# genome/breakdancer

Hardware: AMD Instinct MI355X
Metric: read-pairs/s, records resident in HBM -> scored SV table (SURVEY 8d timing i); end to end from BAM: config.timings.bam_to_table (vs_baseline is taken there) (higher is better)
Workload: dtype int32

## Files before the change

breakdancer_amd/csrc/bdx_api.hip:

```cpp
#include <hip/hip_runtime.h>

#include <algorithm>
#include <atomic>
#include <functional>
#include <memory>
#include <chrono>
#include <cmath>
#include <cstdio>
#include <cstddef>
#include <cstring>
#include <string>
#include <thread>
#include <unordered_map>
#include <utility>
#include <vector>

#include "../../include/bdx.h"
#include "bdx_buf.h"
#include "bdx_dev.h"
#include "bdx_k3.h"
#include "bdx_shard.h"
#include "bdx_scan.h"
#include "bdx_walk.h"
#include "bdx_bam_dev.h"
// ... 15 lines not shown
    DevBuf b_groups;
    DevBuf b_r_rec, b_r_pk, b_out_deg, b_parts, b_rs, b_slot, b_members, b_own, b_lib_stage, b_cn_stage, b_t_lambda, b_t_k, b_ws6;
    DevBuf b_sv_src, b_dlists, b_ltail, b_ins, b_member_ids;
    DevBuf b_sv_out, b_lib_index_out, b_lib_pairs_out, b_cn_key_out, b_cn_value_out, b_ltail_out, b_sv_key;
    PinBuf h_regs, h_pk, h_groups, h_counts0, h_counts2, h_sv_out, h_lib_index, h_lib_pairs, h_cn_key, h_cn_value, h_ltail_dev;
};

constexpr int kNumStages = 12;
enum StageMs { kMsClassify, kMsCompact, kMsCut, kMsJoinAssemble, kMsGroupsWait, kMsHostWalk, kMsFinish, kMsRun, kMsTableWait, kMsMerge, kMsScores };
enum ReadyWord { kPass1Ready, kGroupsReady, kTableReady, kRegionsReady };
constexpr int kK1MaxGrid = 8192;
constexpr uint32_t kK1EventPeriod = 4;

}

struct bdx_ctx {
    int device = 0;
    Stream stream;
    Stream copy_stream;
    bdx_opts opts{};
    std::vector<bdx_lib> libs;
    int nlibs = 0, nbams = 0, ntids = 0, nkeys = 0, w0 = 0;
    std::string err;

    ReadsSoA d{};
    size_t n = 0, cap = 0;
    bool adopted = false;
    DevBuf b_tid, b_pos, b_mtid, b_mpos, b_isize, b_flag, b_qlen, b_mapq, b_lib, b_bam, b_key, b_check;
    bool groups_in_hbm = false;
    bool use_check = false;

    DevBuf b_libs, b_cls, b_tile_tot, b_tile_pre, b_tile_mono, b_blk_cnt, b_cnt, b_p1, b_fold, b_stash, b_chunk_tot, b_counts;
    DevBuf b_lib_mean, b_kdens;
    PinBuf h_p1, h_cnt, h_counts, h_terms;
    PinBuf h_hs_rec, h_hs_aux, h_hs_lists, h_printed;
    StageBufs sb;
    PinBuf h_flags;
    PinBuf h_count;
    uint32_t seq = 0;
    int dbg_no_stash = 0, dbg_max_chunks = 0, dbg_ins_plain = 0, dbg_gather_walk = 0, dbg_regions_copy = 0, dbg_asm_plain = 0, dbg_depth_plain = 0;
    uint32_t lb_seq = 0;
    float k1_ms_last = 0;
    bool k1_timed = false;
    bool stage_timing = false;
    bool poll = true;
    bool materialized = true;
    bool rows_packed = false;
    uint32_t n_sv_total = 0, n_groups_total = 0, n_terms_total = 0, n_cn_total = 0;
    Event ev_groups, ev_regions;
    int big_walk_mode = -1;
    int64_t last_big_groups = -1;
    FinalizeParams fp_deferred{};
    bool finalize2_deferred = false;
    bool bucketed_join = false;
    bool host_walk_only = false;
    K6Arrays k6{};
    const GroupRec* k6_in_groups = nullptr;
    const uint32_t* k6_in_goff = nullptr;
    bool force_direct_join = false;
    uint32_t k6_cap = 0;
    const RegionRec* k6_r_rec = nullptr;
    const uint32_t* k6_r_pk = nullptr;
    uint8_t* k6_taint = nullptr;
    bool table_in_hbm = false;

    bool ran = false;
    Pass1 p1{};
    StageCounts counts{};
    std::vector<uint32_t> cnt;
    std::vector<uint32_t> cnt_local;
    uint32_t g_covered = 0;
    int32_t g_window = 0;
    uint32_t ntiles = 0, tstride = 0;
    Compact cp{};
    K3Arrays k3{};
    K4Arrays k4{};
    std::vector<double> log_tail;
    bool collect_support = false;
    std::vector<uint32_t> ov_cnt;
    uint32_t ov_covered = 0;
    bool replayed = false;
    bool use_stash = false;
    std::atomic<int> sizing{0};
    std::string sizing_err;
    std::vector<uint32_t> sup_off;
    std::vector<uint64_t> sup_idx;
    std::vector<uint8_t> sup_flag;
    std::vector<float> seqcov, lib_density, key_density;
    std::vector<HostRegion> regions;
    std::vector<uint32_t> r_pk;
    const HostRegion* reg = nullptr;
    size_t nreg = 0;
    const uint32_t* rpk = nullptr;
    std::vector<GroupPart> parts;
    WalkResult walk;
    std::unique_ptr<WalkScratch, void (*)(WalkScratch*)> walk_scratch{nullptr, walk_scratch_free};
    uint32_t n_printed = 0;
    uint32_t n_sv_host = 0;
    int speculate = 2;
    int spec_test = 0;
    uint32_t last_na = 0;
    size_t last_n = 0;
    uint32_t count_chunks = 0;
    uint32_t na_alloc = 0;
    bool region_of_fused = false;
    uint32_t join_table_clean = 0;
// ... 510 lines not shown
    }
    launch_kd_apply(p, flag, mask, s);
    HIPCHK(c, hipGetLastError());
    if (h.nwork) {
        HIPCHK(c, hipMemcpyAsync(&h, p.cnt, sizeof(h), hipMemcpyDeviceToHost, s));
        HIPCHK(c, hipStreamSynchronize(s));
        if (h.nlist != h.nwork) return fail(c, BDX_EINTERNAL, "duplicate marking: the work list does not hold the candidates that were counted");
        k.release_long();
    }
    *marked += h.marked; *groups += h.groups;
    return BDX_OK;
}

int mark_duplicates(bdx_ctx* c) {
    if (c->dup_done) return BDX_OK;
    c->dup_marked = 0; c->dup_groups = 0;
    hipStream_t s = c->stream;
    if (c->adopted && (const void*)c->d.flag != c->b_flag.p) {
        HIPCHK(c, c->b_flag.ensure(c->n * 2));
        HIPCHK(c, hipMemcpyAsync(c->b_flag.p, c->d.flag, c->n * 2, hipMemcpyDeviceToDevice, s));
        c->d.flag = c->b_flag.as<uint16_t>();
    }
    KdParams p{};
    p.tid = c->d.tid; p.pos = c->d.pos; p.mtid = c->d.mtid; p.mpos = c->d.mpos; p.flag = c->d.flag;
    p.lib = c->nlibs > 1 ? c->d.lib : nullptr;
    p.key = c->d.key; p.n = c->n;
    size_t ns = 0;
    BDX_TRY(upload_key_segs(c, &ns));
    if (ns) {
        p.nseg = (int)ns;
        p.seg_begin = c->b_seg.as<uint64_t>();
        p.seg_ptr = (const uint64_t* const*)(c->b_seg.as<uint64_t>() + ns + 1);
    }
    BDX_TRY(kd_run(c, p, c->kd, (uint16_t*)c->d.flag, nullptr, s, &c->dup_marked, &c->dup_groups));
    c->dup_done = true;
    return BDX_OK;
}

int pass1_prepare(bdx_ctx* c, uint32_t tiles_cap) {
    HIPCHK(c, hipSetDevice(c->device));
    hipStream_t s = c->stream;
    const int nlibs = c->nlibs, nbams = c->nbams, nkeys = c->nkeys;
    const int ncols = 2 + nkeys, ncnt = nlibs * kNumFlags + nlibs + nbams;
    const uint32_t tstride = (uint32_t)round_up(std::max<uint32_t>(tiles_cap, 16), 16);
    c->tstride = tstride;
    c->k1_cap_tiles = tiles_cap;
    c->k1_done = 0;
    HIPCHK(c, c->b_cls.ensure(std::max<size_t>((size_t)tiles_cap * kTile, 16)));
    c->use_stash = !c->dbg_no_stash && nkeys <= kStashKeys;
    if (c->use_stash) HIPCHK(c, c->b_stash.ensure(std::max<size_t>((size_t)tiles_cap * kStashCap * sizeof(StashRec), 64)));
    HIPCHK(c, c->b_tile_tot.ensure((size_t)ncols * tstride * 4));
    HIPCHK(c, c->b_tile_pre.ensure((size_t)ncols * tstride * 4));
    HIPCHK(c, c->b_tile_mono.ensure((size_t)nbams * tstride * sizeof(MonoRec)));
    HIPCHK(c, c->b_blk_cnt.ensure((size_t)kCntCopies * ncnt * 4));
    HIPCHK(c, c->b_cnt.ensure((size_t)ncnt * 4));
    HIPCHK(c, c->b_p1.ensure(sizeof(Pass1)));
    HIPCHK(c, c->h_p1.ensure(sizeof(Pass1)));
    HIPCHK(c, c->h_cnt.ensure((size_t)ncnt * 4));
    HIPCHK(c, c->h_counts.ensure(sizeof(StageCounts)));
    HIPCHK(c, c->b_counts.ensure(sizeof(StageCounts)));
    HIPCHK(c, c->h_count.ensure((size_t)kMaxChunks * 8));
    const size_t w_tot = (size_t)ncols * tstride, w_mono = (size_t)nbams * tstride * sizeof(MonoRec) / 4;
    if (w_tot > 0xFFFFFFFFull || w_mono > 0xFFFFFFFFull) {
        HIPCHK(c, hipMemsetAsync(c->b_tile_tot.p, 0, w_tot * 4, s));
        HIPCHK(c, hipMemsetAsync(c->b_tile_mono.p, 0xFF, w_mono * 4, s));
    }
    InitList il{};
    int k = 0;
    auto add = [&](void* p, size_t words, uint32_t value) { il.ptr[k] = (uint32_t*)p; il.words[k] = (uint32_t)words; il.value[k] = value; ++k; };
    if (w_tot <= 0xFFFFFFFFull && w_mono <= 0xFFFFFFFFull) { add(c->b_tile_tot.p, w_tot, 0u); add(c->b_tile_mono.p, w_mono, 0xFFFFFFFFu); }
    add(c->b_blk_cnt.p, (size_t)kCntCopies * ncnt, 0u);
    add(c->b_p1.p, sizeof(Pass1) / 4, 0u);
    add(c->b_counts.p, sizeof(StageCounts) / 4, 0u);
    il.n = k;
    launch_init(il, s);
    return BDX_OK;
}

int pass1_classify(bdx_ctx* c, uint32_t upto, bool timed) {
    hipStream_t s = c->stream;
    if (upto <= c->k1_done) return BDX_OK;
    K1Params k1{};
    k1.r = c->d; k1.n = c->n; k1.ntiles = upto; k1.tstride = c->tstride; k1.tile0 = c->k1_done;
    k1.nlibs = c->nlibs; k1.nbams = c->nbams; k1.nkeys = c->nkeys;
    k1.max_sd = c->opts.max_sd; k1.opt_t = c->opts.transchr_rearrange; k1.opt_l = c->opts.illumina_long_insert;
    k1.libs = c->b_libs.as<DevLib>(); k1.cls = c->b_cls.as<uint8_t>(); k1.tile_tot = c->b_tile_tot.as<uint32_t>();
    k1.tile_mono = c->b_tile_mono.as<MonoRec>();
    k1.blk_cnt = c->b_blk_cnt.as<uint32_t>();
    k1.stash = c->use_stash ? c->b_stash.as<StashRec>() : nullptr;
    const uint32_t span = upto - c->k1_done;
    const int grid1 = (int)std::min<uint32_t>((span + kWaves - 1) / kWaves, (uint32_t)kK1MaxGrid);
    launch_k1(k1, grid1, k1_lds_bytes(c->nlibs, c->nbams, c->nkeys), s, timed ? c->ev[0] : nullptr, timed ? c->ev[1] : nullptr);
    c->k1_done = upto;
    return BDX_OK;
}

struct Pass1Launch {
    uint32_t na_cap = 0;
    bool defer_second = false;
    bool post_count = false;
};
int pass1_finalize(bdx_ctx* c, const Pass1Launch& opt) {
    const int nlibs = c->nlibs, nbams = c->nbams, nkeys = c->nkeys;
    const int ncols = 2 + nkeys, ncnt = nlibs * kNumFlags + nlibs + nbams;
    const uint32_t ntiles = c->ntiles;
    FinalizeParams fp{};
    fp.ntiles = ntiles; fp.tstride = c->tstride; fp.nblk = 0;
    fp.nfold = std::max<uint32_t>(1, std::min<uint32_t>(64, (ntiles + 1023) / 1024));
    HIPCHK(c, c->b_fold.ensure((size_t)nbams * fp.nfold * sizeof(MonoRec)));
    fp.fold_part = c->b_fold.as<MonoRec>();
    fp.nlibs = nlibs; fp.nbams = nbams; fp.nkeys = nkeys; fp.ncols = ncols; fp.ncnt = ncnt; fp.w0 = c->w0;
    fp.tile_tot = c->b_tile_tot.as<uint32_t>(); fp.tile_pre = c->b_tile_pre.as<uint32_t>(); fp.tile_mono = c->b_tile_mono.as<MonoRec>();
    {
        const uint32_t nsuper = (ntiles + kK2TilesPerWave - 1) / kK2TilesPerWave;
        const uint32_t round = 4096;
        const uint32_t rounds = std::max<uint32_t>(1, (nsuper + round - 1) / round);
        const uint32_t max_chunks = c->dbg_max_chunks > 0 ? (uint32_t)std::min(c->dbg_max_chunks, (int)kMaxChunks) : (uint32_t)kMaxChunks;
        fp.chunk_super = round * ((rounds + max_chunks - 1) / max_chunks);
        fp.nchunk = std::max<uint32_t>(1, (nsuper + fp.chunk_super - 1) / fp.chunk_super);
        HIPCHK(c, c->b_chunk_tot.ensure((size_t)ncols * kMaxChunks * 8));
        fp.chunk_tot = c->b_chunk_tot.as<uint32_t>();
        fp.chunk_base = fp.chunk_tot + (size_t)ncols * kMaxChunks;
    }
    fp.blk_cnt = c->b_blk_cnt.as<uint32_t>(); fp.cnt = c->b_cnt.as<uint32_t>(); fp.p1 = c->b_p1.as<Pass1>();
    HIPCHK(c, c->b_kdens.ensure(64 * 4));
    fp.libs = c->b_libs.as<DevLib>(); fp.cn_lib = c->opts.cn_lib; fp.key_density = c->b_kdens.as<float>();
    fp.cnt_host = c->h_cnt.as<uint32_t>(); fp.p1_host = c->h_p1.as<Pass1>();
    memset(c->h_p1.p, 0, sizeof(Pass1));
    HIPCHK(c, c->h_flags.ensure(64));
    ++c->seq;
    fp.flag_host = c->h_flags.as<uint32_t>(); fp.flag_value = c->seq;
    fp.na_cap = opt.na_cap;
    fp.count_host = opt.post_count && c->poll ? c->h_count.as<uint64_t>() : nullptr; fp.count_stamp = c->seq;
    c->count_chunks = fp.count_host ? fp.nchunk : 0;
    c->fp_deferred = fp;
    c->finalize2_deferred = opt.defer_second;
    launch_finalize(fp, c->stream, !opt.defer_second);
    return BDX_OK;
}

int do_pass1(bdx_ctx* c, const Pass1Launch& opt) {
    HIPCHK(c, hipSetDevice(c->device));
    hipStream_t s = c->stream;
    if (c->n >= ((size_t)1 << 32)) return fail(c, BDX_ELIMIT, "more than 2^32 - 1 reads in one context (read indices and the prefix counters are 32-bit)");
    const uint32_t ntiles = (uint32_t)((c->n + kTile - 1) / kTile);
    c->ntiles = ntiles;
    c->ran = false; c->replayed = false;
    c->cls_n = (size_t)-1;
    c->na_alloc = 0;
    c->regions.clear(); c->r_pk.clear(); c->parts.clear();
    c->reg = nullptr; c->nreg = 0; c->rpk = nullptr;
    c->walk.clear();
    if (!c->walk_scratch) c->walk_scratch.reset(walk_scratch_new());
    c->n_printed = 0;
    memset(&c->counts, 0, sizeof(c->counts));
    for (float& m : c->stage_ms) m = 0;

    if (c->copy_pending) {
        HIPCHK(c, hipStreamWaitEvent(s, c->ev_copy, 0));
        c->copy_pending = false;
    }
    if (!(c->k1_live && c->k1_cap_tiles >= ntiles)) {
        BDX_TRY(pass1_prepare(c, ntiles));
    }
    c->k1_live = false;
    if (c->mark_dup && c->k1_done == 0) {
        BDX_TRY(mark_duplicates(c));
    }
    const bool time_k1 = (c->stage_timing || c->seq % kK1EventPeriod == 0) && c->k1_done == 0 && ntiles > 0;
    BDX_TRY(pass1_classify(c, ntiles, time_k1));
    BDX_TRY(pass1_finalize(c, opt));
    c->k1_timed = time_k1;
    return BDX_OK;
}

int wait_pass1(bdx_ctx* c) {
    const int ncnt = c->nlibs * kNumFlags + c->nlibs + c->nbams;
    BDX_TRY(await_ready(c, kPass1Ready, nullptr, "the pass-1 record did not arrive: its kernel was not launched", true));
    c->p1 = *c->h_p1.as<Pass1>();
    c->cnt_local.assign(c->h_cnt.as<uint32_t>(), c->h_cnt.as<uint32_t>() + ncnt);
    if (c->k1_timed) {
        float ms = 0;
        if (hipEventElapsedTime(&ms, c->ev[0], c->ev[1]) == hipSuccess) c->k1_ms_last = ms;
    }
    c->stage_ms[kMsClassify] = c->k1_ms_last;
    if (c->p1.n_anom > kMaxAnomalous) return fail(c, BDX_ELIMIT, "more than 2^31 anomalous reads in one context");
    if (!c->na_alloc && c->p1.n_anom) c->na_alloc = (uint32_t)std::min<uint64_t>(with_headroom(c->p1.n_anom), kMaxAnomalous);
    c->cls_n = c->n;
    return BDX_OK;
}

int32_t window_from(const bdx_ctx* c, const uint32_t* cnt, uint32_t covered) {
    int W = c->w0;
    for (int i = 0; i < c->nlibs; ++i) {
        const int nd = (int)(cnt[i * kNumFlags + F_LARGE] + cnt[i * kNumFlags + F_SMALL]);
        const int tmp = nd > 0 ? (int)((float)covered / (float)nd) : 50;
        W = std::min(W, tmp);
    }
    return W;
}

int set_pass1(bdx_ctx* c, const uint32_t* cnt, uint32_t covered, int32_t window, bool upload) {
    const int nlibs = c->nlibs, nkeys = c->nkeys;
    const int ncnt = nlibs * kNumFlags + nlibs + c->nbams;
    c->cnt.assign(cnt, cnt + ncnt);
    c->g_covered = covered;
    c->g_window = window;
    const uint32_t* lib_cnt = c->cnt.data() + nlibs * kNumFlags;
    const uint32_t* bam_cnt = lib_cnt + nlibs;
    c->seqcov.assign(nlibs, 0.f);
    c->lib_density.assign(nlibs, 0.f);
    c->key_density.assign(nkeys, 0.000001f);
    for (int i = 0; i < nlibs; ++i) {
        float covg = 0;
        if (lib_cnt[i] != 0 && covered != 0) covg = float(lib_cnt[i]) * c->libs[i].readlens / covered;
        c->seqcov[i] = covg;
        float dens = 0.000001f;
        if (c->opts.cn_lib) {
            if (lib_cnt[i] != 0) dens = float(lib_cnt[i]) / covered;
        } else {
            dens = float(bam_cnt[c->libs[i].bam_index]) / covered;
        }
        c->lib_density[i] = dens;
        c->key_density[c->opts.cn_lib ? i : c->libs[i].bam_index] = dens;
    }
    struct { uint32_t covered; int32_t window; } hdr{covered, window};
    static_assert(offsetof(Pass1, covered_ref_len) == 0 && offsetof(Pass1, window) == 4, "Pass1 header layout");
    if (upload) {
        HIPCHK(c, hipMemcpyAsync(c->b_p1.p, &hdr, sizeof(hdr), hipMemcpyHostToDevice, c->stream));
        HIPCHK(c, hipStreamSynchronize(c->stream));
    }
// ... 93 lines not shown
    SZCHK(b.b_cn_stage.ensure(cap * (size_t)d.nkeys * sizeof(CnStage) + 16));
    SZCHK(b.b_t_lambda.ensure((size_t)k.term * 8)); SZCHK(b.b_t_k.ensure((size_t)k.term * 4));
    if (d.table_in_hbm) {
        SZCHK(b.b_sv_out.ensure((size_t)k.sv * sizeof(SvOut))); SZCHK(b.b_sv_key.ensure((size_t)k.sv * 8));
        SZCHK(b.b_lib_index_out.ensure((size_t)k.term * 4)); SZCHK(b.b_lib_pairs_out.ensure((size_t)k.term * 4));
        SZCHK(b.b_cn_key_out.ensure((size_t)k.cn * 4 + 16)); SZCHK(b.b_cn_value_out.ensure((size_t)k.cn * 4 + 16));
        SZCHK(b.b_ltail_out.ensure((size_t)k.term * 8));
    } else {
        SZCHK(b.h_sv_out.ensure((size_t)k.sv * sizeof(SvOut)));
        SZCHK(b.h_lib_index.ensure((size_t)k.term * 4)); SZCHK(b.h_lib_pairs.ensure((size_t)k.term * 4));
        SZCHK(b.h_cn_key.ensure((size_t)k.cn * 4 + 16)); SZCHK(b.h_cn_value.ensure((size_t)k.cn * 4 + 16));
        SZCHK(b.h_ltail_dev.ensure((size_t)k.term * 8));
    }
    SZCHK(b.h_counts2.ensure(sizeof(StageCounts)));
    SZCHK(b.b_sv_src.ensure((size_t)k.sv * 16)); SZCHK(b.b_ltail.ensure((size_t)k.term * 8));
    SZCHK(b.b_dlists.ensure((size_t)k.term * 4 + (size_t)k.cn * 8 + 64));
    SZCHK(b.b_ins.ensure(k.p2 * 12 + (size_t)k.sv * 8 + ((size_t)k.sv + 1) * 16 + k.nsort * 12 + k.nsort * 4 * kK6RankSlices + 64));
    SZCHK(size_zero_once(b.b_ws6, 4 * (scan_grid((uint32_t)cap, 1) + 1) * 8, s));
    return BDX_OK;
}

int do_compact(bdx_ctx* c) {
    HIPCHK(c, hipSetDevice(c->device));
    hipStream_t s = c->stream;
    const int nkeys = c->nkeys;
    const uint32_t na = c->na_alloc;
    if (c->stage_timing) HIPCHK(c, hipEventRecord(c->ev[2], s));
    Compact& cp = c->cp;
    cp = Compact{};
    c->k3 = K3Arrays{};
    if (na) {
        const StageDims dm = stage_dims(c, na);
        BDX_TRY(size_compact(c->sb, dm, &c->err));
        const StageBufs& b = c->sb;
        cp.tid = b.b_c_tid.as<int32_t>(); cp.pos = b.b_c_pos.as<int32_t>(); cp.isize = b.b_c_isize.as<int32_t>();
        cp.meta = b.b_c_meta.as<uint32_t>(); cp.key = b.b_c_key.as<uint64_t>(); cp.nn = b.b_c_nn.as<uint32_t>();
        cp.idx = b.b_c_idx.as<uint32_t>();
        cp.check = c->use_check ? b.b_c_check.as<uint64_t>() : nullptr;
        cp.pk = b.b_c_pk.as<uint32_t>(); cp.cap = na;
        K2Params k2{};
        k2.r = c->d; k2.n = c->n; k2.ntiles = c->ntiles; k2.tstride = c->tstride; k2.nkeys = nkeys; k2.nlibs = c->nlibs; k2.libs = c->b_libs.as<DevLib>();
        k2.cls = c->b_cls.as<uint8_t>(); k2.tile_pre = c->b_tile_pre.as<uint32_t>(); k2.c = cp;
        k2.tile_tot = c->b_tile_tot.as<uint32_t>(); k2.stash = c->use_stash ? c->b_stash.as<StashRec>() : nullptr;
        k2.chunk_tot = c->fp_deferred.chunk_tot; k2.chunk_base = c->fp_deferred.chunk_base; k2.chunk_super = c->fp_deferred.chunk_super;
        k2.fill_ptr[0] = b.b_c_maxq.as<uint32_t>(); k2.fill_words[0] = na; k2.fill_value[0] = 0u;
        c->join_table_clean = 0;
        if (dm.k2_clears_join) {
            const uint32_t slots = dm.join_slots;
            k2.fill_ptr[1] = b.b_t_key.as<uint32_t>(); k2.fill_words[1] = 2 * slots; k2.fill_value[1] = 0xFFFFFFFFu;
            k2.fill_ptr[2] = b.b_partner.as<uint32_t>(); k2.fill_words[2] = na; k2.fill_value[2] = 0xFFFFFFFFu;
            k2.fill_ptr[3] = b.b_pair_lo.as<uint32_t>(); k2.fill_words[3] = na; k2.fill_value[3] = 0xFFFFFFFFu;
            c->join_table_clean = slots;
        }
        {
            size_t ns = 0;
            BDX_TRY(upload_key_segs(c, &ns));
            if (ns) {
                k2.nseg = (int)ns;
                k2.seg_begin = c->b_seg.as<uint64_t>();
                k2.seg_ptr = (const uint64_t* const*)(c->b_seg.as<uint64_t>() + ns + 1);
                k2.seg_qlen = (const uint16_t* const*)(c->b_seg.as<uint64_t>() + 2 * ns + 1);
                k2.seg_check = (const uint64_t* const*)(c->b_seg.as<uint64_t>() + 3 * ns + 1);
            }
        }
        launch_k2(k2, k2_lds_bytes(nkeys), s, c->finalize2_deferred ? &c->fp_deferred : nullptr);
        c->finalize2_deferred = false;
    }
    if (c->finalize2_deferred) {
        launch_finalize2_only(c->fp_deferred, s);
        c->finalize2_deferred = false;
    }
    if (c->stage_timing) HIPCHK(c, hipEventRecord(c->ev[3], s));
    return BDX_OK;
}

void own_borrowed_regions(bdx_ctx* c) {
    if (!c->reg || (const void*)c->reg != c->sb.h_regs.p) return;
    const HostRegion* r = c->reg;
    const uint32_t* pk = c->rpk;
    const size_t n = c->nreg;
    std::vector<HostRegion> keep(r, r + n);
    std::vector<uint32_t> keep_pk;
    if (pk) keep_pk.assign(pk, pk + n * 2 * (size_t)c->nkeys);
    c->regions.swap(keep); c->r_pk.swap(keep_pk);
    c->reg = c->regions.data(); c->rpk = c->r_pk.data();
}

int do_cut(bdx_ctx* c, const uint32_t* tid_tail, RegionDst dst) {
    HIPCHK(c, hipSetDevice(c->device));
    hipStream_t s = c->stream;
    const uint32_t na = c->na_alloc;
    if (na) {
        StageDims dm = stage_dims(c, na);
        dm.regions = dst;
        BDX_TRY(size_cut(c->sb, dm, s, &c->err));
        const StageBufs& b = c->sb;
        K3Arrays& k3 = c->k3;
        const bool for_k6 = dst == RegionDst::HostAndHbm;
        k3.cap = na;
        k3.cand = b.b_cand.as<int32_t>(); k3.pre_q = b.b_pre_q.as<uint32_t>(); k3.pre_rev = b.b_pre_rev.as<uint32_t>();
        k3.pre_nonctx = b.b_pre_nonctx.as<uint32_t>(); k3.c_first = b.b_c_first.as<uint32_t>();
        k3.c_maxq = b.b_c_maxq.as<int32_t>(); k3.c_rid = b.b_c_rid.as<int32_t>(); k3.region_of = b.b_region_of.as<int32_t>();
        k3.r_rec = for_k6 ? b.h_regs.as<RegionRec>() : b.b_r_rec.as<RegionRec>();
        k3.r_pk = for_k6 ? b.h_pk.as<uint32_t>() : b.b_r_pk.as<uint32_t>();
        if (for_k6) {
            k3.r_rec_dev = b.b_r_rec.as<RegionRec>(); k3.r_pk_dev = b.b_r_pk.as<uint32_t>(); k3.out_deg = b.b_out_deg.as<uint32_t>();
            k3.host_copy_later = joins_direct(c, na) ? 1 : 0;
            memset(b.h_counts0.p, 0, sizeof(StageCounts));
            k3.counts_host = b.h_counts0.as<StageCounts>();
        } else {
            k3.r_rec_dev = nullptr; k3.r_pk_dev = nullptr; k3.host_copy_later = 0;
        }
        k3.lb_state = b.b_lb.as<unsigned long long>();
        HIPCHK(c, next_lb_stamp(c, &k3.lb_stamp));
        k3.counts = c->b_counts.as<StageCounts>();
        c->region_of_fused = for_k6 && joins_direct(c, na);
        launch_k3(k3, c->cp, c->b_p1.as<Pass1>(), na, c->opts.min_len, c->opts.seq_coverage_lim, c->nkeys, tid_tail, !c->region_of_fused, s);
        if (for_k6 && !k3.host_copy_later) {
            BDX_TRY(signal_ready(c, kRegionsReady, c->ev_regions));
// ... 468 lines not shown
        en.cand = c->k3.cand; en.c_rid = c->k3.c_rid; en.region_out = c->k3.region_of;
        en.k6_scratch = c->k3.out_deg; en.scratch_cap = c->k3.cap;
        if (c->k3.host_copy_later) {
            en.r_rec_dev = c->k3.r_rec_dev; en.r_pk_dev = c->k3.r_pk_dev; en.r_rec_host = c->k3.r_rec; en.r_pk_host = c->k3.r_pk;
            en.counts = c->b_counts.as<StageCounts>(); en.nkeys2 = 2 * c->nkeys;
        }
    }
    BDX_TRY(do_join_local(c, c->na_alloc, en, &c->b_p1.as<Pass1>()->n_anom));
    if (c->k3.host_copy_later && !c->poll) {
        BDX_TRY(signal_ready(c, kRegionsReady, c->ev_regions));
    }
    BDX_TRY(k6_prepare(c, force_host, 0));
    return k6_then_walk(c, launch_k6_groups);
}

enum class Sizing { Restored, Ahead, Exact };
struct SizingPlan { Sizing route; uint32_t guess; };

SizingPlan plan_sizing(const bdx_ctx* c) {
    if (!c->ov_cnt.empty()) return {Sizing::Restored, 0};
    uint64_t guess = 0;
    if (c->speculate == 2 && c->ran && c->last_n == c->n && c->last_na) {
        guess = c->spec_test ? std::max(1u, c->last_na / 2) : with_headroom(c->last_na);
    } else if (c->speculate && c->n >= (1u << 20) && (c->speculate == 1 || c->n < (1u << 25))) {
        guess = prior_anomalous(c->n, c->spec_test ? 4096 : 32);
    }
    if (!guess || guess > kMaxAnomalous) return {Sizing::Exact, 0};
    return {Sizing::Ahead, (uint32_t)guess};
}

int adopt_own_pass1(bdx_ctx* c) { return set_pass1(c, c->cnt_local.data(), c->p1.covered_ref_len, c->p1.window, false); }

int run_restored(bdx_ctx* c, bool force_host) {
    hipStream_t s = c->stream;
    BDX_TRY(do_pass1(c, {}));
    BDX_TRY(wait_pass1(c));
    BDX_TRY(set_pass1(c, c->ov_cnt.data(), c->ov_covered, window_from(c, c->ov_cnt.data(), c->ov_covered), true));
    HIPCHK(c, hipMemcpyAsync(c->b_cnt.p, c->ov_cnt.data(), c->ov_cnt.size() * 4, hipMemcpyHostToDevice, s));
    HIPCHK(c, hipMemcpyAsync(c->b_kdens.p, c->key_density.data(), c->key_density.size() * 4, hipMemcpyHostToDevice, s));
    HIPCHK(c, hipStreamSynchronize(s));
    return enqueue_middle(c, force_host);
}

int run_ahead(bdx_ctx* c, uint32_t guess, bool force_host) {
    hipStream_t s = c->stream;
    BDX_TRY(do_pass1(c, {.na_cap = guess, .defer_second = true}));
    c->na_alloc = guess;
    BDX_TRY(enqueue_middle(c, force_host));
    BDX_TRY(wait_pass1(c));
    BDX_TRY(adopt_own_pass1(c));
    if (c->p1.n_anom <= guess) return BDX_OK;
    HIPCHK(c, hipStreamSynchronize(s));
    HIPCHK(c, hipMemcpy(&c->b_p1.as<Pass1>()->n_anom, &c->p1.n_anom, 4, hipMemcpyHostToDevice));
    HIPCHK(c, hipMemset(c->b_counts.p, 0, sizeof(StageCounts)));
    ++c->seq;
    c->na_alloc = c->p1.n_anom;
    return enqueue_middle(c, force_host);
}

int run_exact(bdx_ctx* c, bool force_host) {
    hipStream_t s = c->stream;
    BDX_TRY(do_pass1(c, {.post_count = true}));
    uint64_t count = 0;
    if (!wait_count(c, &count)) {
        BDX_TRY(wait_pass1(c));
        BDX_TRY(adopt_own_pass1(c));
        return enqueue_middle(c, force_host);
    }
    if (count > kMaxAnomalous) {
        HIPCHK(c, hipStreamSynchronize(s));
        return fail(c, BDX_ELIMIT, "more than 2^31 anomalous reads in one context");
    }
    if (count) c->na_alloc = (uint32_t)std::min<uint64_t>(with_headroom(count), kMaxAnomalous);
    BDX_TRY(enqueue_middle(c, force_host));
    BDX_TRY(wait_pass1(c));
    if (c->p1.n_anom != count) {
        HIPCHK(c, hipStreamSynchronize(s));
        return fail(c, BDX_EINTERNAL, "the count of anomalous reads posted ahead of the pass-1 record differs from the record's");
    }
    return adopt_own_pass1(c);
}

int enqueue_device_half(bdx_ctx* c, const SizingPlan& plan, bool force_host) {
    hipStream_t s = c->stream;
    switch (plan.route) {
        case Sizing::Restored: BDX_TRY(run_restored(c, force_host)); break;
        case Sizing::Ahead: BDX_TRY(run_ahead(c, plan.guess, force_host)); break;
        case Sizing::Exact: BDX_TRY(run_exact(c, force_host)); break;
    }
    c->last_n = c->n;
    c->last_na = c->p1.n_anom;
    if (c->stage_timing) HIPCHK(c, hipEventRecord(c->ev[5], s));
    return BDX_OK;
}

int receive_regions_and_groups(bdx_ctx* c, uint32_t ph) {
    hipStream_t s = c->stream;
    BDX_TRY(await_ready(c, kRegionsReady, c->ev_regions, "the region table did not arrive: its kernels were not launched"));
    const uint32_t nr_host = c->sb.h_counts0.as<StageCounts>()->n_regions;
    if ((uint64_t)nr_host + ph > kMaxRegions) {
        HIPCHK(c, hipStreamSynchronize(s));
        return fail(c, BDX_ELIMIT, "more than 2^26 - 2 accepted regions in one context");
    }
    const bool copy_first = c->dbg_regions_copy == 1 || (c->dbg_regions_copy == 0 && nr_host < kBorrowRegionsMin);
    if (copy_first) decode_regions(c, c->sb.h_regs.as<RegionRec>(), c->sb.h_pk.as<uint32_t>(), nr_host, ph, false);
    BDX_TRY(await_ready(c, kGroupsReady, c->ev_groups, "the pair groups did not arrive: their kernels were not launched"));
    c->counts = *c->h_counts.as<StageCounts>();
// ... 498 lines not shown
```

breakdancer_amd/csrc/bdx_dev.h:

```cpp
#pragma once
#include <hip/hip_runtime.h>
#include <stdint.h>

namespace bdx {

constexpr int kTile = 256;
constexpr int kBlock = 256;
constexpr int kWaves = kBlock / 64;
constexpr int kNumFlags = 11;
constexpr int kK2TilesPerWave = 4;
constexpr int kCntCopies = 64;
constexpr int kMaxChunks = 64;
constexpr int kStashCap = 16;
constexpr int kStashKeys = 2;

struct StashRec {
    int32_t tid, pos, isize;
    uint32_t meta;
    uint32_t where;
    uint32_t proper;
    uint32_t pad[2];
};
static_assert(sizeof(StashRec) == 32, "two 16-byte stores");

// ... 7 lines not shown
};

struct ReadsSoA {
    const int32_t *tid, *pos, *mtid, *mpos, *isize;
    const uint16_t *flag, *qlen;
    const uint8_t *mapq, *lib, *bam;
    const uint64_t* key;
    const uint64_t* check;
};

struct MonoRec {
    int32_t ft, fp, lt, lp;
    long long sum;
};

constexpr int kColAnom = 0, kColNormal = 1, kColKey0 = 2;

struct K1Params {
    ReadsSoA r;
    uint64_t n;
    uint32_t ntiles, tstride;
    uint32_t tile0;
    int nlibs, nbams, nkeys;
    int max_sd, opt_t, opt_l;
    const DevLib* libs;
    uint8_t* cls;
    uint32_t* tile_tot;
    MonoRec* tile_mono;
    uint32_t* blk_cnt;
    StashRec* stash;
};

struct Pass1 {
    uint32_t covered_ref_len;
    int32_t window;
    uint32_t n_anom;
    uint32_t n_normal;
    uint32_t key_tot[60];
    unsigned long long ref_len[256];
};

struct FinalizeParams {
    uint32_t ntiles, tstride, nblk;
    uint32_t nfold;
    MonoRec* fold_part;
    int nlibs, nbams, nkeys, ncols, ncnt;
    int w0;
    const uint32_t* tile_tot;
    uint32_t* tile_pre;
    uint32_t* chunk_tot;
    uint32_t* chunk_base;
    uint32_t chunk_super, nchunk;
    const MonoRec* tile_mono;
    const uint32_t* blk_cnt;
    uint32_t* cnt;
    Pass1* p1;
    uint32_t* cnt_host;
    Pass1* p1_host;
    const DevLib* libs;
    int cn_lib;
    float* key_density;
    uint32_t* flag_host;
    uint32_t flag_value;
    uint64_t* count_host;
    uint32_t count_stamp;
    uint32_t na_cap;
};

struct InitList {
    uint32_t* ptr[6];
    uint32_t words[6];
    uint32_t value[6];
    int n;
};
void launch_init(const InitList& l, hipStream_t s);

struct Compact {
    int32_t* tid;
    int32_t* pos;
    int32_t* isize;
    uint32_t* meta;
    uint64_t* key;
    uint64_t* check;
    uint32_t* idx;
    uint32_t* nn;
    uint32_t* pk;
    uint32_t cap;
};

struct K2Params {
    ReadsSoA r;
    uint64_t n;
    uint32_t ntiles, tstride;
    int nkeys, nlibs;
    const DevLib* libs;
    const uint8_t* cls;
    const uint32_t* tile_pre;
    const uint32_t* chunk_tot;
    const uint32_t* chunk_base;
    uint32_t chunk_super;
    const uint32_t* tile_tot;
    const StashRec* stash;
    Compact c;
    uint32_t* fill_ptr[4];
    uint32_t fill_words[4];
    uint32_t fill_value[4];
    int nseg;
    const uint64_t* seg_begin;
    const uint64_t* const* seg_ptr;
    const uint16_t* const* seg_qlen;
    const uint64_t* const* seg_check;
};

__device__ __forceinline__ uint32_t meta_pack(int flag, int rev, int lib, int qlen) {
    return (uint32_t)flag | ((uint32_t)rev << 4) | ((uint32_t)lib << 8) | ((uint32_t)qlen << 16);
}
__host__ __device__ __forceinline__ int meta_flag(uint32_t m) { return m & 15; }
__host__ __device__ __forceinline__ int meta_rev(uint32_t m) { return (m >> 4) & 1; }
__host__ __device__ __forceinline__ int meta_lib(uint32_t m) { return (m >> 8) & 255; }
__host__ __device__ __forceinline__ int meta_qlen(uint32_t m) { return m >> 16; }

__device__ __forceinline__ int lane_id() { return threadIdx.x & 63; }
__device__ __forceinline__ int wave_id() { return threadIdx.x >> 6; }
__device__ __forceinline__ uint64_t ballot64(bool p) { return __builtin_amdgcn_ballot_w64(p); }
__device__ __forceinline__ int popc64(uint64_t m) { return __popcll(m); }

__device__ __forceinline__ uint32_t wave_incl_scan(uint32_t v) {
    const int l = lane_id();
#pragma unroll
    for (int o = 1; o < 64; o <<= 1) {
        uint32_t t = __shfl_up(v, o);
        if (l >= o) v += t;
    }
    return v;
}

struct StoreView {
    const int32_t *tid, *pos, *mtid, *mpos, *isize;
    const uint16_t* flag;
    const uint8_t* cls;
    uint64_t n;
};

struct K8Params {
    StoreView st;
    const uint8_t* key;
    const int32_t *q_tid, *q_a, *q_b;
    uint32_t nq;
    int nkeys;
    int32_t lmax;
    uint32_t* counts;
};

struct KsSite {
    int32_t tid1, pos1, tid2, pos2;
    uint32_t flag_mask;
};
struct KsParams {
    StoreView st;
// ... 81 lines not shown
```

breakdancer_amd/csrc/bdx_finalize.h:

```cpp
#pragma once
#include <cstddef>

#include "bdx_dev.h"

namespace bdx {

__device__ __forceinline__ MonoRec mono_combine(const MonoRec& a, const MonoRec& b) {
    if (a.ft == -1) return b;
    if (b.ft == -1) return a;
    MonoRec r;
    r.ft = a.ft; r.fp = a.fp; r.lt = b.lt; r.lp = b.lp;
    r.sum = a.sum + b.sum + (a.lt == b.ft ? (long long)b.fp - (long long)a.lp : 0ll);
    return r;
}
__device__ __forceinline__ MonoRec mono_shfl_down(const MonoRec& a, int o) {
    MonoRec r;
    r.ft = __shfl_down(a.ft, o); r.fp = __shfl_down(a.fp, o); r.lt = __shfl_down(a.lt, o); r.lp = __shfl_down(a.lp, o);
    r.sum = __shfl_down(a.sum, o);
    return r;
}

__device__ __forceinline__ void finalize2_body(const FinalizeParams& p) {
    __shared__ uint32_t s_acc[255 * 12 + 256];
    __shared__ unsigned long long s_ref[256];
    __shared__ uint32_t s_head[2];
    __shared__ uint32_t s_col[64];
    const int t = threadIdx.x, lane = t & 63, w = t >> 6;
    for (int i = t; i < p.ncnt; i += 256) s_acc[i] = 0;
    __syncthreads();
    for (int idx = t; idx < kCntCopies * p.ncnt; idx += 256) {
        const uint32_t v = p.blk_cnt[idx];
        if (v) atomicAdd(&s_acc[idx % p.ncnt], v);
    }
    __syncthreads();
    for (int i = t; i < p.ncnt; i += 256) {
        const uint32_t v = s_acc[i];
        p.cnt[i] = v;
        if (p.cnt_host) p.cnt_host[i] = v;
    }
    for (int c0 = 0; c0 < p.ncols; c0 += 4) {
        const int c = c0 + w;
        uint32_t v = (c < p.ncols && (uint32_t)lane < p.nchunk) ? p.chunk_tot[(size_t)c * kMaxChunks + lane] : 0u;
        {
            uint32_t inc = v;
#pragma unroll
            for (int o = 1; o < 64; o <<= 1) {
                const uint32_t u = __shfl_up(inc, o);
                if (lane >= o) inc += u;
            }
            if (c < p.ncols) p.chunk_base[(size_t)c * kMaxChunks + lane] = inc - v;
        }
#pragma unroll
        for (int o = 32; o > 0; o >>= 1) v += __shfl_xor(v, o);
        if (lane == 0 && c < p.ncols) {
            s_col[c] = v;
            if (c == kColAnom) p.p1->n_anom = v;
            else if (c == kColNormal) p.p1->n_normal = v;
            else p.p1->key_tot[c - kColKey0] = v;
        }
    }
    for (int b0 = 0; b0 < p.nbams; b0 += 4) {
        const int b = b0 + w;
        MonoRec acc;
        acc.ft = -1; acc.fp = 0; acc.lt = 0; acc.lp = 0; acc.sum = 0;
        if (b < p.nbams && (uint32_t)lane < p.nfold) acc = p.fold_part[(size_t)b * p.nfold + lane];
#pragma unroll
        for (int o = 1; o < 64; o <<= 1) {
            const MonoRec other = mono_shfl_down(acc, o);
            if (lane + o < 64 && ((lane & (2 * o - 1)) == 0)) acc = mono_combine(acc, other);
        }
        if (lane == 0 && b < p.nbams) {
            const unsigned long long r = acc.ft == -1 ? 0ull : (unsigned long long)acc.sum;
            s_ref[b] = r;
            p.p1->ref_len[b] = r;
        }
    }
    __syncthreads();
    if (t == 0) {
        uint32_t covered = 0;
        for (int b = 0; b < p.nbams; ++b)
            if ((unsigned long long)covered < s_ref[b]) covered = (uint32_t)s_ref[b];
        p.p1->covered_ref_len = covered;
        int W = p.w0;
        for (int i = 0; i < p.nlibs; ++i) {
            const int nd = (int)(s_acc[i * kNumFlags + F_LARGE] + s_acc[i * kNumFlags + F_SMALL]);
// ... 50 lines not shown
```

breakdancer_amd/csrc/k1_classify.hip:

```cpp
#include <cstddef>

#include <hip/hip_ext.h>

#include "bdx_dev.h"
#include "bdx_finalize.h"

#include <limits.h>

#ifdef BDX_KPROF
#include "bdx_scan.h"
#else
#define KPROF(row, col) do {} while (0)
#endif

namespace bdx {

constexpr int kMixedLibs = 8;

typedef int v4i __attribute__((ext_vector_type(4)));
typedef unsigned short v4us __attribute__((ext_vector_type(4)));
typedef unsigned char v4uc __attribute__((ext_vector_type(4)));
__device__ __forceinline__ int4 ldnt(const int32_t* p) { const v4i v = __builtin_nontemporal_load((const v4i*)p); return make_int4(v.x, v.y, v.z, v.w); }
__device__ __forceinline__ ushort4 ldnt(const uint16_t* p) { const v4us v = __builtin_nontemporal_load((const v4us*)p); return make_ushort4(v.x, v.y, v.z, v.w); }
__device__ __forceinline__ uchar4 ldnt(const uint8_t* p) { const v4uc v = __builtin_nontemporal_load((const v4uc*)p); return make_uchar4(v.x, v.y, v.z, v.w); }
// ... 554 lines not shown
                }
                if (lane_m == 0)
                    for (int b = 0; b < nbams_m; ++b)
                        if (my_mono[b].ft != -1) p.tile_mono[(size_t)b * p.tstride + tile] = my_mono[b];
            }
            }
        }
    }
    __syncthreads();
    uint32_t* out = p.blk_cnt + (size_t)(blockIdx.x & (kCntCopies - 1)) * ncnt;
    for (int i = t; i < ncnt; i += kBlock) {
        const uint32_t v = s_cnt[i];
        if (v) atomicAdd(&out[i], v);
    }
}

void launch_k1(const K1Params& p, int grid, size_t lds, hipStream_t s, hipEvent_t start, hipEvent_t stop) {
    auto kernel = p.opt_l ? k1_classify_kernel<true> : k1_classify_kernel<false>;
    if (start && stop) hipExtLaunchKernelGGL(kernel, dim3(grid), dim3(kBlock), (uint32_t)lds, s, start, stop, 0u, p);
    else hipLaunchKernelGGL(kernel, dim3(grid), dim3(kBlock), lds, s, p);
}

constexpr int kFinBlock = 1024;

__global__ __launch_bounds__(kFinBlock) void finalize_kernel(const FinalizeParams p) {
    __shared__ uint32_t s_carry;
    __shared__ MonoRec s_mono[kFinBlock / 64];
    const int t = threadIdx.x, lane = t & 63, w = t >> 6;
    KPROF(blockIdx.x * 16 + w, 0);

    const uint32_t nscan = (uint32_t)p.ncols * p.nchunk;
    if (blockIdx.x < nscan) {
        const int c = (int)(blockIdx.x / p.nchunk);
        const uint32_t g = blockIdx.x % p.nchunk;
        const uint32_t tile_lo = g * p.chunk_super * kK2TilesPerWave;
        const uint32_t tile_hi = min(p.ntiles, (g + 1) * p.chunk_super * kK2TilesPerWave);
        const uint32_t* in = p.tile_tot + (size_t)c * p.tstride;
        uint32_t* out = p.tile_pre + (size_t)c * p.tstride;
        if (t == 0) s_carry = 0;
        __syncthreads();
        constexpr int kQ = 4;
        static_assert(kK2TilesPerWave == 4 && kFinBlock == 1024, "one 16-byte load per super tile");
        __shared__ uint32_t s_wt[kQ * (kFinBlock / 64)];
        __shared__ uint32_t s_round;
        const uint32_t row_hi = min(p.tstride, (g + 1) * p.chunk_super * kK2TilesPerWave);
        volatile uint64_t* const count_word = (c == kColAnom && t == 0 && p.count_host) ? p.count_host + g : nullptr;
        if (count_word && tile_lo >= tile_hi) *count_word = (uint64_t)p.count_stamp << 32;
        for (uint32_t base = tile_lo; base < tile_hi; base += kFinBlock * kQ * 4) {
            uint32_t sum[kQ], inc[kQ];
#pragma unroll
            for (int q = 0; q < kQ; ++q) {
                const uint32_t i = base + ((uint32_t)q * kFinBlock + t) * 4;
                uint4 x = make_uint4(0, 0, 0, 0);
                if (i < row_hi) x = *(const uint4*)(in + i);
                sum[q] = x.x + x.y + x.z + x.w;
            }
            if (sum[0] != 0xFFFFFFFFu) KPROF(blockIdx.x * 16 + w, 1);
#pragma unroll
            for (int q = 0; q < kQ; ++q) inc[q] = wave_incl_scan(sum[q]);
            if (lane == 63) {
#pragma unroll
                for (int q = 0; q < kQ; ++q) s_wt[q * (kFinBlock / 64) + w] = inc[q];
            }
            __syncthreads();
            if (w == 0) {
                static_assert(kQ * (kFinBlock / 64) == 64, "one wave total per lane");
                const uint32_t v = s_wt[lane];
                const uint32_t li = wave_incl_scan(v);
                s_wt[lane] = li - v;
                if (lane == 63) s_round = li;
            }
            __syncthreads();
            if (count_word && tile_hi - base <= (uint32_t)(kFinBlock * kQ * 4)) *count_word = ((uint64_t)p.count_stamp << 32) | (uint32_t)(s_carry + s_round);
#pragma unroll
            for (int q = 0; q < kQ; ++q) {
                const uint32_t i = base + ((uint32_t)q * kFinBlock + t) * 4;
                if (i < row_hi) out[i / 4] = s_carry + s_wt[q * (kFinBlock / 64) + w] + inc[q] - sum[q];
            }
            __syncthreads();
            if (t == 0) s_carry += s_round;
            __syncthreads();
        }
        if (t == 0) p.chunk_tot[(size_t)c * kMaxChunks + g] = s_carry;
        KPROF(blockIdx.x * 16 + w, 2);
        return;
    }

    const uint32_t fb = blockIdx.x - nscan;
    const uint32_t chunk = (p.ntiles + p.nfold - 1) / p.nfold;
    const uint32_t c0 = fb * chunk, c1 = min(c0 + chunk, p.ntiles);
    const uint32_t per = (chunk + kFinBlock - 1) / kFinBlock;
    for (int b = 0; b < p.nbams; ++b) {
        const MonoRec* mo = p.tile_mono + (size_t)b * p.tstride;
        MonoRec acc;
        acc.ft = -1; acc.fp = 0; acc.lt = 0; acc.lp = 0; acc.sum = 0;
        const uint32_t t0 = min(c0 + (uint32_t)t * per, c1), t1 = min(t0 + per, c1);
        for (uint32_t i = t0; i < t1; i += 8) {
            MonoRec e[8];
#pragma unroll
            for (int q = 0; q < 8; ++q) {
                if (i + q < t1) e[q] = mo[i + q];
                else e[q].ft = -1;
            }
#pragma unroll
            for (int q = 0; q < 8; ++q) acc = mono_combine(acc, e[q]);
        }
        if (acc.ft != -12345) KPROF(blockIdx.x * 16 + w, 1);
// ... 53 lines not shown
```

breakdancer_amd/csrc/k2_compact.hip:

```cpp
#include <cstdlib>

#include "bdx_dev.h"
#include "bdx_finalize.h"

namespace bdx {

size_t k2_lds_bytes(int) { return 0; }

constexpr int kSub = kK2TilesPerWave;
constexpr int kPerLane = 4 * kSub;
constexpr int kTile2 = kTile * kSub;
constexpr int kSlice = 256;
constexpr int kOffBits = 10;
static_assert(kPerLane <= 32 && kTile2 <= (1 << kOffBits), "K2 super tile");

__device__ __forceinline__ unsigned class_byte(const uint64_t (&cq)[kSub / 2], int r) {
    uint64_t v = cq[0];
#pragma unroll
    for (int q = 1; q < kSub / 2; ++q) v = (r >> 3) == q ? cq[q] : v;
    return (unsigned)((v >> (8 * (r & 7))) & 255u);
}

__device__ __forceinline__ void key_and_qlen_of(const K2Params& p, uint64_t i, uint64_t& key, int& qlen, uint64_t& check) {
    if (p.nseg == 0) {
// ... 158 lines not shown
                    const unsigned sam = p.r.flag[i];
                    p.c.tid[j] = p.r.tid[i];
                    p.c.pos[j] = p.r.pos[i];
                    p.c.isize[j] = abs(p.r.isize[i]);
                    uint64_t key, check = 0;
                    int qlen;
                    key_and_qlen_of(p, i, key, qlen, check);
                    p.c.meta[j] = meta_pack((int)((src >> kOffBits) & 15u), (sam >> 4) & 1u, lib_of(p, i), qlen);
                    p.c.key[j] = key;
                    if (p.c.check) p.c.check[j] = check;
                    p.c.idx[j] = (uint32_t)i;
                    p.c.nn[j] = s_nn[w * kSlice + q];
                }
            }
            __builtin_amdgcn_wave_barrier();
        }
        uint64_t kq[kSub / 2];
#pragma unroll
        for (int q = 0; q < kSub / 2; ++q) kq[q] = 0;
        if (nkeys > 1) {
#pragma unroll
            for (int r = 0; r < kPerLane; ++r)
                if (r < nvalid) kq[r >> 3] |= (uint64_t)(p.libs[lib_of(p, base + r)].key & 255) << (8 * (r & 7));
        }
        for (int k0 = 0; k0 < nkeys; k0 += 2) {
            uint32_t mk0 = 0, mk1 = 0;
            if (nkeys > 1) {
#pragma unroll
                for (int r = 0; r < kPerLane; ++r) {
                    const int key = (int)((kq[r >> 3] >> (8 * (r & 7))) & 255u);
                    if ((m_pk >> r) & 1u) { mk0 |= key == k0 ? 1u << r : 0u; mk1 |= key == k0 + 1 ? 1u << r : 0u; }
                }
            } else {
                mk0 = m_pk;
            }
            const uint32_t v = (uint32_t)__popc(mk0) + ((uint32_t)__popc(mk1) << 16);
            const uint32_t ex = wave_incl_scan(v) - v;
            const uint32_t b0 = k0 == 0 ? pre_k0 : col_prefix<kBases>(p, kColKey0 + k0, tile2, chunk, lane);
            const uint32_t b1 = k0 + 1 < nkeys ? (k0 == 0 ? pre_k1 : col_prefix<kBases>(p, kColKey0 + k0 + 1, tile2, chunk, lane)) : 0u;
            uint32_t j = rank0 + local0;
            for (uint32_t mm = m_anom; mm; mm &= mm - 1, ++j) {
                if (j >= p.c.cap) break;
                const int r = __builtin_ctz(mm);
                const uint32_t upto = (2u << r) - 1u;
                p.c.pk[(size_t)k0 * p.c.cap + j] = b0 + (ex & 0xFFFFu) + (uint32_t)__popc(mk0 & upto);
                if (k0 + 1 < nkeys) p.c.pk[(size_t)(k0 + 1) * p.c.cap + j] = b1 + (ex >> 16) + (uint32_t)__popc(mk1 & upto);
            }
        }
    }
}

__device__ __forceinline__ void k2_fills(const K2Params& p) {
#pragma nounroll
    for (int f = 0; f < 4; ++f)
        for (uint32_t i = blockIdx.x * kBlock + threadIdx.x; i < p.fill_words[f]; i += gridDim.x * kBlock) p.fill_ptr[f][i] = p.fill_value[f];
}

__global__ __launch_bounds__(kBlock) void k2_compact_kernel(const K2Params p) {
    k2_fills(p);
    k2_body<true>(p, gridDim.x);
}

__global__ __launch_bounds__(kBlock) void k2_compact_side_kernel(const K2Params p, const FinalizeParams fp) {
    k2_fills(p);
    if (blockIdx.x == gridDim.x - 1) {
        finalize2_body(fp);
        return;
    }
    k2_body<false>(p, gridDim.x - 1);
}

void launch_k2(const K2Params& p, size_t lds, hipStream_t s, const FinalizeParams* side) {
    const uint32_t ntiles2 = (p.ntiles + kSub - 1) / kSub;
    const uint32_t nblk = (ntiles2 + kWaves - 1) / kWaves;
    const uint32_t cap = 8192u;
    const uint32_t grid = nblk < cap ? nblk : cap;
    if (side) hipLaunchKernelGGL(k2_compact_side_kernel, dim3(grid + 1), dim3(kBlock), lds, s, p, *side);
    else hipLaunchKernelGGL(k2_compact_kernel, dim3(grid), dim3(kBlock), lds, s, p);
}

}

__global__ void k2_noop_kernel() {}
namespace bdx { void warm_k2(hipStream_t s) { hipLaunchKernelGGL(k2_noop_kernel, dim3(1), dim3(64), 0, s); } }
```

Baseline: 29.59 billion.

## Skip redundant pass-1 buffer initialisation and fold counter resets into kernels

Stops zeroing the per-tile total table and, for single-BAM inputs, the mono table each run. The finalize kernel now reads tiles masked to the tile bound instead of the row bound. The per-block counters are cleared by the finalize kernel as it consumes them, so the init pass skips them when they are known clean. The StageCounts reset moves into the K2 fill list (or a tiny init launch), removing a synchronous hipMemset. Host-side container clears are moved after the K1 launch so they overlap with GPU work. The risk is correctness if the tile_tot entries are not fully rewritten by K1 or the clean-flag tracking goes stale.

New measurement: 29.45 billion. No clear change (-0.5%).

```diff
diff --git a/breakdancer_amd/csrc/bdx_api.hip b/breakdancer_amd/csrc/bdx_api.hip
--- a/breakdancer_amd/csrc/bdx_api.hip
+++ b/breakdancer_amd/csrc/bdx_api.hip
@@ -91,6 +91,7 @@
     int64_t last_big_groups = -1;
     FinalizeParams fp_deferred{};
     bool finalize2_deferred = false;
+    bool blk_cnt_clean = false;
     bool bucketed_join = false;
     bool host_walk_only = false;
     K6Arrays k6{};
@@ -707,6 +708,7 @@
     HIPCHK(c, c->b_tile_tot.ensure((size_t)ncols * tstride * 4));
     HIPCHK(c, c->b_tile_pre.ensure((size_t)ncols * tstride * 4));
     HIPCHK(c, c->b_tile_mono.ensure((size_t)nbams * tstride * sizeof(MonoRec)));
+    if (c->b_blk_cnt.bytes < (size_t)kCntCopies * ncnt * 4) c->blk_cnt_clean = false;
     HIPCHK(c, c->b_blk_cnt.ensure((size_t)kCntCopies * ncnt * 4));
     HIPCHK(c, c->b_cnt.ensure((size_t)ncnt * 4));
     HIPCHK(c, c->b_p1.ensure(sizeof(Pass1)));
@@ -715,18 +717,15 @@
     HIPCHK(c, c->h_counts.ensure(sizeof(StageCounts)));
     HIPCHK(c, c->b_counts.ensure(sizeof(StageCounts)));
     HIPCHK(c, c->h_count.ensure((size_t)kMaxChunks * 8));
-    const size_t w_tot = (size_t)ncols * tstride, w_mono = (size_t)nbams * tstride * sizeof(MonoRec) / 4;
-    if (w_tot > 0xFFFFFFFFull || w_mono > 0xFFFFFFFFull) {
-        HIPCHK(c, hipMemsetAsync(c->b_tile_tot.p, 0, w_tot * 4, s));
-        HIPCHK(c, hipMemsetAsync(c->b_tile_mono.p, 0xFF, w_mono * 4, s));
-    }
     InitList il{};
     int k = 0;
     auto add = [&](void* p, size_t words, uint32_t value) { il.ptr[k] = (uint32_t*)p; il.words[k] = (uint32_t)words; il.value[k] = value; ++k; };
-    if (w_tot <= 0xFFFFFFFFull && w_mono <= 0xFFFFFFFFull) { add(c->b_tile_tot.p, w_tot, 0u); add(c->b_tile_mono.p, w_mono, 0xFFFFFFFFu); }
-    add(c->b_blk_cnt.p, (size_t)kCntCopies * ncnt, 0u);
-    add(c->b_p1.p, sizeof(Pass1) / 4, 0u);
-    add(c->b_counts.p, sizeof(StageCounts) / 4, 0u);
+    if (nbams > 1) {
+        const size_t w_mono = (size_t)nbams * tstride * sizeof(MonoRec) / 4;
+        if (w_mono > 0xFFFFFFFFull) HIPCHK(c, hipMemsetAsync(c->b_tile_mono.p, 0xFF, w_mono * 4, s));
+        else add(c->b_tile_mono.p, w_mono, 0xFFFFFFFFu);
+    }
+    if (!c->blk_cnt_clean) add(c->b_blk_cnt.p, (size_t)kCntCopies * ncnt, 0u);
     il.n = k;
     launch_init(il, s);
     return BDX_OK;
@@ -745,6 +744,7 @@
     k1.stash = c->use_stash ? c->b_stash.as<StashRec>() : nullptr;
     const uint32_t span = upto - c->k1_done;
     const int grid1 = (int)std::min<uint32_t>((span + kWaves - 1) / kWaves, (uint32_t)kK1MaxGrid);
+    c->blk_cnt_clean = false;
     launch_k1(k1, grid1, k1_lds_bytes(c->nlibs, c->nbams, c->nkeys), s, timed ? c->ev[0] : nullptr, timed ? c->ev[1] : nullptr);
     c->k1_done = upto;
     return BDX_OK;
@@ -803,13 +803,8 @@
     c->ran = false; c->replayed = false;
     c->cls_n = (size_t)-1;
     c->na_alloc = 0;
-    c->regions.clear(); c->r_pk.clear(); c->parts.clear();
     c->reg = nullptr; c->nreg = 0; c->rpk = nullptr;
-    c->walk.clear();
-    if (!c->walk_scratch) c->walk_scratch.reset(walk_scratch_new());
     c->n_printed = 0;
-    memset(&c->counts, 0, sizeof(c->counts));
-    for (float& m : c->stage_ms) m = 0;
 
     if (c->copy_pending) {
         HIPCHK(c, hipStreamWaitEvent(s, c->ev_copy, 0));
@@ -824,6 +819,11 @@
     }
     const bool time_k1 = (c->stage_timing || c->seq % kK1EventPeriod == 0) && c->k1_done == 0 && ntiles > 0;
     BDX_TRY(pass1_classify(c, ntiles, time_k1));
+    c->regions.clear(); c->r_pk.clear(); c->parts.clear();
+    c->walk.clear();
+    if (!c->walk_scratch) c->walk_scratch.reset(walk_scratch_new());
+    memset(&c->counts, 0, sizeof(c->counts));
+    for (float& m : c->stage_ms) m = 0;
     BDX_TRY(pass1_finalize(c, opt));
     c->k1_timed = time_k1;
     return BDX_OK;
@@ -832,6 +832,7 @@
 int wait_pass1(bdx_ctx* c) {
     const int ncnt = c->nlibs * kNumFlags + c->nlibs + c->nbams;
     BDX_TRY(await_ready(c, kPass1Ready, nullptr, "the pass-1 record did not arrive: its kernel was not launched", true));
+    c->blk_cnt_clean = true;
     c->p1 = *c->h_p1.as<Pass1>();
     c->cnt_local.assign(c->h_cnt.as<uint32_t>(), c->h_cnt.as<uint32_t>() + ncnt);
     if (c->k1_timed) {
@@ -1031,6 +1032,7 @@
             k2.fill_ptr[3] = b.b_pair_lo.as<uint32_t>(); k2.fill_words[3] = na; k2.fill_value[3] = 0xFFFFFFFFu;
             c->join_table_clean = slots;
         }
+        k2.fill_ptr[4] = c->b_counts.as<uint32_t>(); k2.fill_words[4] = sizeof(StageCounts) / 4; k2.fill_value[4] = 0u;
         {
             size_t ns = 0;
             BDX_TRY(upload_key_segs(c, &ns));
@@ -1044,6 +1046,10 @@
         }
         launch_k2(k2, k2_lds_bytes(nkeys), s, c->finalize2_deferred ? &c->fp_deferred : nullptr);
         c->finalize2_deferred = false;
+    } else {
+        InitList il{};
+        il.ptr[0] = c->b_counts.as<uint32_t>(); il.words[0] = sizeof(StageCounts) / 4; il.value[0] = 0u; il.n = 1;
+        launch_init(il, s);
     }
     if (c->finalize2_deferred) {
         launch_finalize2_only(c->fp_deferred, s);
@@ -1618,7 +1624,6 @@
     if (c->p1.n_anom <= guess) return BDX_OK;
     HIPCHK(c, hipStreamSynchronize(s));
     HIPCHK(c, hipMemcpy(&c->b_p1.as<Pass1>()->n_anom, &c->p1.n_anom, 4, hipMemcpyHostToDevice));
-    HIPCHK(c, hipMemset(c->b_counts.p, 0, sizeof(StageCounts)));
     ++c->seq;
     c->na_alloc = c->p1.n_anom;
     return enqueue_middle(c, force_host);
diff --git a/breakdancer_amd/csrc/bdx_dev.h b/breakdancer_amd/csrc/bdx_dev.h
--- a/breakdancer_amd/csrc/bdx_dev.h
+++ b/breakdancer_amd/csrc/bdx_dev.h
@@ -83,7 +83,7 @@
     uint32_t* chunk_base;
     uint32_t chunk_super, nchunk;
     const MonoRec* tile_mono;
-    const uint32_t* blk_cnt;
+    uint32_t* blk_cnt;
     uint32_t* cnt;
     Pass1* p1;
     uint32_t* cnt_host;
@@ -119,6 +119,7 @@
     uint32_t cap;
 };
 
+constexpr int kK2Fills = 5;
 struct K2Params {
     ReadsSoA r;
     uint64_t n;
@@ -133,9 +134,9 @@
     const uint32_t* tile_tot;
     const StashRec* stash;
     Compact c;
-    uint32_t* fill_ptr[4];
-    uint32_t fill_words[4];
-    uint32_t fill_value[4];
+    uint32_t* fill_ptr[kK2Fills];
+    uint32_t fill_words[kK2Fills];
+    uint32_t fill_value[kK2Fills];
     int nseg;
     const uint64_t* seg_begin;
     const uint64_t* const* seg_ptr;
diff --git a/breakdancer_amd/csrc/bdx_finalize.h b/breakdancer_amd/csrc/bdx_finalize.h
--- a/breakdancer_amd/csrc/bdx_finalize.h
+++ b/breakdancer_amd/csrc/bdx_finalize.h
@@ -30,7 +30,10 @@
     __syncthreads();
     for (int idx = t; idx < kCntCopies * p.ncnt; idx += 256) {
         const uint32_t v = p.blk_cnt[idx];
-        if (v) atomicAdd(&s_acc[idx % p.ncnt], v);
+        if (v) {
+            atomicAdd(&s_acc[idx % p.ncnt], v);
+            p.blk_cnt[idx] = 0u;
+        }
     }
     __syncthreads();
     for (int i = t; i < p.ncnt; i += 256) {
diff --git a/breakdancer_amd/csrc/k1_classify.hip b/breakdancer_amd/csrc/k1_classify.hip
--- a/breakdancer_amd/csrc/k1_classify.hip
+++ b/breakdancer_amd/csrc/k1_classify.hip
@@ -630,7 +630,12 @@
             for (int q = 0; q < kQ; ++q) {
                 const uint32_t i = base + ((uint32_t)q * kFinBlock + t) * 4;
                 uint4 x = make_uint4(0, 0, 0, 0);
-                if (i < row_hi) x = *(const uint4*)(in + i);
+                if (i < tile_hi) {
+                    x = *(const uint4*)(in + i);
+                    if (i + 1 >= tile_hi) x.y = 0;
+                    if (i + 2 >= tile_hi) x.z = 0;
+                    if (i + 3 >= tile_hi) x.w = 0;
+                }
                 sum[q] = x.x + x.y + x.z + x.w;
             }
             if (sum[0] != 0xFFFFFFFFu) KPROF(blockIdx.x * 16 + w, 1);
diff --git a/breakdancer_amd/csrc/k2_compact.hip b/breakdancer_amd/csrc/k2_compact.hip
--- a/breakdancer_amd/csrc/k2_compact.hip
+++ b/breakdancer_amd/csrc/k2_compact.hip
@@ -234,7 +234,7 @@
 
 __device__ __forceinline__ void k2_fills(const K2Params& p) {
 #pragma nounroll
-    for (int f = 0; f < 4; ++f)
+    for (int f = 0; f < kK2Fills; ++f)
         for (uint32_t i = blockIdx.x * kBlock + threadIdx.x; i < p.fill_words[f]; i += gridDim.x * kBlock) p.fill_ptr[f][i] = p.fill_value[f];
 }
 
```
